# gicheonkang/gst-visdial

Hardware: AMD Instinct MI355X
Metric: dialog-rounds/sec (enc_dec_a train step) (higher is better)
Workload: dtype bf16; 1 GPU; enc_dec_a train step (fwd+loss+bwd+allreduce+AdamW, dropout on), 16 rows/GPU, seq_len 256, 37x2048 region features, answer len 25 [BASELINE configs[1] per-GPU shape]; global_batch=16, rows_per_gpu=16, seq_len=256, parallelism=dp1, hip_graph=True, optimizer_update=in the weight-gradient launch's epilogue + remainder pass, payload_written_by_wgrad_launch=False, capture_quiesce=no-process-group, full=False

## Files before the change

### gst_visdial_amd/_lib.py

```python
import ctypes as C
import os

_HERE = os.path.dirname(os.path.abspath(__file__))
LIB_PATH = os.path.join(_HERE, "lib", "libgstvd_hip.so")
ABI_VERSION = 9

F32, BF16 = 0, 1
COS_TOPK_AUTO, COS_TOPK_MANY, COS_TOPK_FEW = 0, 1, 2
EPI_BIAS, EPI_ADD, EPI_GELU, EPI_DGELU, EPI_DROPOUT = 1, 2, 4, 8, 16
EPI_COLSUM, EPI_COLSUM_ACC = 32, 64
EPI_ADAMW = 128
LN_RESID, LN_EMBED, LN_IMAGE = 0, 1, 2
RANK_MAX_OPTIONS = 128
(RANK_N_SPARSE, RANK_N_GT_SKIPPED, RANK_N_NDCG, RANK_N_NDCG_EMPTY, RANK_N_REL_SKIPPED, RANK_N_CALLS, RANK_NDCG_SUM) = range(7)
RANK_HIST = 8
RANK_ACC_SLOTS = RANK_HIST + RANK_MAX_OPTIONS + 1

_vp, _i64, _i32, _f32, _u32 = C.c_void_p, C.c_int64, C.c_int32, C.c_float, C.c_uint32


class GemmDesc(C.Structure):
    _fields_ = [("A", _vp), ("B", _vp), ("C", _vp), ("bias", _vp), ("addend", _vp), ("aux", _vp),
                ("M", _i64), ("N", _i64), ("K", _i64),
                ("lda", _i64), ("ldb", _i64), ("ldc", _i64), ("ldadd", _i64), ("ldaux", _i64),
# ... 150 lines not shown
    "gstvd_gemm_ln_bwd": (_i32, [C.POINTER(GemmDesc), C.POINTER(LnBwdDesc), _vp]),
    "gstvd_gemm_ln_rows_per_block": (_i64, []),
    "gstvd_colsum_partials": (_i32, [_vp, _i64, _i64, _i64, _vp, _vp, _vp, _i32, _vp]),
    "gstvd_colsum_batched": (_i32, [_vp, _i64, _i64, _vp]),
    "gstvd_colsum_slabs_batched": (_i32, [_vp, _i64, _i64, _i32, _vp]),
    "gstvd_colsum_slabs": (_i32, [_vp, _i64, _i64, _i64, _i32, _vp, _i64, _vp]),
    "gstvd_colsum": (_i32, [_vp, _i64, _i64, _i64, _i32, _vp, _vp, _i64, _i32, _vp]),
    "gstvd_locgrad": (_i32, [_vp, _i64, _vp, _i64, _i64, _i32, _vp, _i32, _vp]),
    "gstvd_attn_fwd": (_i32, [C.POINTER(AttnDesc), _vp]),
    "gstvd_attn_bwd": (_i32, [C.POINTER(AttnDesc), _vp]),
    "gstvd_attn_group_bwd": (_i32, [C.POINTER(AttnDesc), _vp]),
    "gstvd_ln_kernel_name": (_i32, [_vp, _i32, C.c_char_p, _i32]),
    "gstvd_attn_kernel_name": (_i32, [C.POINTER(AttnDesc), _i32, C.c_char_p, _i32]),
    "gstvd_attn_probs": (_i32, [C.POINTER(AttnDesc), _vp, _i32, _vp]),
    "gstvd_ce_fwd": (_i32, [_vp, _i64, _vp, _i64, _i64, _i64, _i32, _vp, _vp, _vp, _vp]),
    "gstvd_ce_bwd": (_i32, [_vp, _i64, _vp, _vp, _vp, _vp, _i32, _i64, _i64, _i64, _i32, _vp, _i64, _vp]),
    "gstvd_ce_bwd_rows": (_i32, [_vp, _i64, _vp, _vp, _vp, _i64, _i64, _i64, _i32, _vp, _i64, _vp]),
    "gstvd_fgsm_step": (_i32, [_vp, _vp, _f32, _vp, _i64, _vp]),
    "gstvd_answer_scores": (_i32, [_vp, _i64, _vp, _vp, _i64, _i64, _i32, _vp, _vp]),
    "gstvd_rank_loss": (_i32, [_vp, _i64, _vp, _vp, _vp, _i64, _i64, _i64, _f32, _i32, _vp, _vp, _vp, _vp, _vp, _vp]),
    "gstvd_sample_topk": (_i32, [C.POINTER(SampleDesc), _vp]),
    "gstvd_sample_topk_scored": (_i32, [C.POINTER(SampleDesc), _vp, _i64, _vp]),
    "gstvd_vl_split": (_i32, [_vp, _i64, _i64, _i64, _i64, _i32, _vp, _vp, _f32, _u32, _u32, _vp, _vp]),
    "gstvd_cast": (_i32, [_vp, _i32, _vp, _i32, _i64, _vp]),
    "gstvd_cast_ranges": (_i32, [_vp, _vp, _vp, _vp, _i64, _i64, _vp]),
    "gstvd_scale": (_i32, [_vp, _vp, _i64, _vp]),
    "gstvd_rng_advance": (_i32, [_vp, _vp]),
    "gstvd_dropout_mask": (_i32, [_vp, _i64, _f32, _u32, _vp, _vp]),
    "gstvd_adamw": (_i32, [_vp, _vp, _vp, _vp, _vp, _i64, _vp, _vp, _i64, _f32, _f32, _f32, _vp, _f32, _i64, _vp]),
    "gstvd_adamw_bf16grad": (_i32, [_vp, _vp, _i64, _vp, _vp, _vp, _i64, _vp, _vp, _i64, _f32, _f32, _f32, _vp, _f32, _i64, _vp]),
# ... 73 lines not shown
```

### gst_visdial_amd/csrc/layernorm.hip

```cpp
#include <stdio.h>

#include "common.h"

struct LnP {
  gstvd_ln_t f;
  const void* dy; int64_t lddy; void* dres; int64_t lddres; void* dx; int64_t lddx; float* partial;
  float *dword, *dpos, *dtt, *dtt_ext;
};

static inline int ln_bwd_rw(int64_t M) { return M <= 8192 ? 1 : 2; }
static inline int ln_bwd_nw(int64_t M, int mode, int64_t H) { return (M >= 2048 && mode != GSTVD_LN_EMBED && H <= 768) ? 16 : 4; }

template <typename T, int MODE>
DEVFN f32x4 ln_prologue(const gstvd_ln_t& f, int64_t row, int c, const DropKey& dpre,
                        int64_t id, int64_t tpos, int64_t seg, const float* locrow) {
  f32x4 h;
  if (MODE == GSTVD_LN_RESID) {
    h = ld4((const T*)f.x + row * f.ldx + c);
    h *= drop_factor4(dpre, (uint64_t)(row * f.H + c));
    if (f.res) h += ld4((const T*)f.res + row * f.ldres + c);
  } else if (MODE == GSTVD_LN_EMBED) {
    h = *(const f32x4*)(f.word + id * f.H + c) + *(const f32x4*)(f.pos + tpos * f.H + c);
    const float* trow = (seg < f.type_vocab) ? f.tt + seg * f.H : f.tt_ext + (seg - f.type_vocab) * f.H;
    h += *(const f32x4*)(trow + c);
// ... 521 lines not shown
  if (dtype == GSTVD_BF16) hipLaunchKernelGGL(colsum_slab_kernel<bf16>, grid, dim3(256), 0, s, (const bf16*)x, ldx, M, N, scratch);
  else if (dtype == GSTVD_F32) hipLaunchKernelGGL(colsum_slab_kernel<float>, grid, dim3(256), 0, s, (const float*)x, ldx, M, N, scratch);
  else return GSTVD_E_DTYPE;
  GSTVD_LAUNCH_CHECK();
  hipLaunchKernelGGL(colsum_final_kernel, dim3((unsigned)((N + 63) / 64)), dim3(256), 0, s, scratch, nslab, N, out, accumulate);
  GSTVD_LAUNCH_CHECK();
  return 0;
}

extern "C" int gstvd_locgrad(const void* dh, int64_t lddh, const float* loc, int64_t M, int64_t H, int32_t dtype,
                             float* dw_loc, int32_t accumulate, gstvd_stream_t stream) {
  if (!dh || !loc || !dw_loc) return GSTVD_E_NULL;
  if (M <= 0 || H <= 0) return GSTVD_E_SHAPE;
  hipStream_t s = (hipStream_t)stream;
  if (!accumulate) {
    hipError_t e = hipMemsetAsync(dw_loc, 0, (size_t)H * 5 * sizeof(float), s);
    if (e != hipSuccess) return (int)e;
  }
  dim3 grid((unsigned)((H + 255) / 256), 16);
  if (dtype == GSTVD_BF16) hipLaunchKernelGGL(locgrad_kernel<bf16>, grid, dim3(256), 0, s, (const bf16*)dh, lddh, loc, M, H, dw_loc);
  else if (dtype == GSTVD_F32) hipLaunchKernelGGL(locgrad_kernel<float>, grid, dim3(256), 0, s, (const float*)dh, lddh, loc, M, H, dw_loc);
  else return GSTVD_E_DTYPE;
  GSTVD_LAUNCH_CHECK();
  return 0;
}
```

### gst_visdial_amd/csrc/loss.hip

```cpp
#include "loss_reduce.h"
#include "ce_row.h"
#include <math.h>

template <typename T>
__global__ __launch_bounds__(256) void ce_fwd_kernel(const T* logits, int64_t ldl, const int64_t* labels, int64_t V,
                                                     int64_t ignore, float* row_loss, float* lse_out) {
  __shared__ float red[4];
  const int64_t m = blockIdx.x;
  const T* x = logits + m * ldl;
  const int64_t V4 = V & ~(int64_t)3;
  float mx = -INFINITY;
  for (int64_t c = threadIdx.x * 4; c < V4; c += 1024) {
    f32x4 v = ld4(x + c);
    mx = fmaxf(fmaxf(mx, fmaxf(v[0], v[1])), fmaxf(v[2], v[3]));
  }
  for (int64_t c = V4 + threadIdx.x; c < V; c += 256) mx = fmaxf(mx, to_f(x[c]));
  mx = block_reduce(mx, red, true);
  float s = 0.f;
  for (int64_t c = threadIdx.x * 4; c < V4; c += 1024) {
    f32x4 v = ld4(x + c);
    s += __expf(v[0] - mx) + __expf(v[1] - mx) + __expf(v[2] - mx) + __expf(v[3] - mx);
  }
  for (int64_t c = V4 + threadIdx.x; c < V; c += 256) s += __expf(to_f(x[c]) - mx);
  s = block_reduce(s, red, false);
  if (threadIdx.x == 0) {
    const float lse = mx + logf(s);
    lse_out[m] = lse;
    const int64_t lab = labels[m];
    row_loss[m] = (lab == ignore || lab < 0 || lab >= V) ? 0.f : lse - to_f(x[lab]);
  }
}

template <typename T>
__global__ __launch_bounds__(256) void ce_bwd_kernel(const T* logits, int64_t ldl, const int64_t* labels, const float* lse,
                                                     const float* stats, const float* gscale, int mean, int64_t V,
                                                     int64_t ignore, T* dl, int64_t ldd) {
  const int64_t m = blockIdx.x;
  const int64_t lab = labels[m];
  const bool keep = !(lab == ignore || lab < 0 || lab >= V);
  float gs = gscale ? gscale[0] : 1.f;
  if (mean) gs /= stats[1];
  ce_bwd_row(logits + m * ldl, dl + m * ldd, lab, keep, lse[m], gs, V, ldd);
}

template <typename T>
// ... 189 lines not shown
  GSTVD_FOR_DTYPE(dtype, E, hipLaunchKernelGGL(vl_split_kernel<E>, grid, dim3(256), 0, s, (const E*)d_enc, B, R, T, H, (E*)d_v, (E*)d_t, p, site_v, site_t, rng));
  GSTVD_LAUNCH_CHECK();
  return 0;
}

extern "C" int gstvd_abi_version(void) { return 9; }
extern "C" const char* gstvd_build_arch(void) { return "gfx950"; }

extern "C" int gstvd_ce_fwd(const void* logits, int64_t ldl, const int64_t* labels, int64_t M, int64_t V, int64_t ignore_index,
                            int32_t dtype, float* row_loss, float* lse, float* stats, gstvd_stream_t stream) {
  if (!logits || !labels || !row_loss || !lse || !stats) return GSTVD_E_NULL;
  if (M <= 0 || V <= 0 || (ldl % 4) || ldl < V) return GSTVD_E_SHAPE;
  if (dtype != GSTVD_BF16 && dtype != GSTVD_F32) return GSTVD_E_DTYPE;
  if (ce_misaligned(logits, dtype)) return GSTVD_E_ALIGN;
  hipStream_t s = (hipStream_t)stream;
  GSTVD_FOR_DTYPE(dtype, T, hipLaunchKernelGGL(ce_fwd_kernel<T>, dim3((unsigned)M), dim3(256), 0, s, (const T*)logits, ldl, labels, V, ignore_index, row_loss, lse));
  GSTVD_LAUNCH_CHECK();
  hipLaunchKernelGGL(row_loss_reduce_kernel, dim3(1), dim3(256), 0, s, (const float*)row_loss, labels, ignore_index, 0, M, stats);
  GSTVD_LAUNCH_CHECK();
  return 0;
}

extern "C" int gstvd_ce_bwd(const void* logits, int64_t ldl, const int64_t* labels, const float* lse, const float* stats,
                            const float* gscale, int32_t mean, int64_t M, int64_t V, int64_t ignore_index, int32_t dtype,
                            void* dlogits, int64_t ldd, gstvd_stream_t stream) {
  if (!logits || !labels || !lse || !stats || !dlogits) return GSTVD_E_NULL;
  if (M <= 0 || V <= 0 || (ldl % 4) || (ldd % 4) || ldl < V || ldd < V) return GSTVD_E_SHAPE;
  if (dtype != GSTVD_BF16 && dtype != GSTVD_F32) return GSTVD_E_DTYPE;
  if (ce_misaligned(logits, dtype) || ce_misaligned(dlogits, dtype)) return GSTVD_E_ALIGN;
  hipStream_t s = (hipStream_t)stream;
  GSTVD_FOR_DTYPE(dtype, T, hipLaunchKernelGGL(ce_bwd_kernel<T>, dim3((unsigned)M), dim3(256), 0, s, (const T*)logits, ldl, labels, lse, stats, gscale, mean, V, ignore_index, (T*)dlogits, ldd));
  GSTVD_LAUNCH_CHECK();
  return 0;
// ... 131 lines not shown
```

### gst_visdial_amd/csrc/loss_reduce.h

```cpp
#pragma once
#include "common.h"

static __global__ __launch_bounds__(256) void row_loss_reduce_kernel(const float* row_loss, const int64_t* labels, int64_t value, int eq,
                                                                     int64_t M, float* stats) {
  __shared__ float red[4];
  float s = 0.f, n = 0.f;
  for (int64_t i = threadIdx.x; i < M; i += blockDim.x) {
    s += row_loss[i];
    n += (!labels || (labels[i] == value) == (eq != 0)) ? 1.f : 0.f;
  }
  s = block_reduce(s, red, false);
  n = block_reduce(n, red, false);
  if (threadIdx.x == 0) { stats[0] = s; stats[1] = n; stats[2] = s / n; }
}
```

### gst_visdial_amd/engine.py

```python
import contextlib
import os
import weakref

import torch

from . import attn_maps, ops
from .config import encoder_schedule
from .engine_decode import DecodeMixin
from .engine_disc import DiscMixin, _DiscFn
from .engine_rank import RankMixin, _RankFn
from .storage import Act, Arena, FlatParams
from ._lib import GstvdError, EPI_GELU, EPI_DGELU, LN_RESID, LN_EMBED, LN_IMAGE


EARLY_WGRAD = 1

_DEVICE_STREAMS = {}


def device_streams(device):
    key = torch.device(device).index
    if key is None:
        key = torch.cuda.current_device()
    if key not in _DEVICE_STREAMS:
# ... 14 lines not shown
        self.enc_cfg, self.dec_cfg = enc_cfg, dec_cfg
        prec = params.get("amd_precision", "bf16")
        if prec not in ("bf16", "fp32"):
            raise GstvdError("params['amd_precision'] must be 'bf16' or 'fp32'")
        self.precision = prec
        self.adt = torch.bfloat16 if prec == "bf16" else torch.float32
        self.flat = None
        self.arena = None
        self.rng = None
        self._decode_sessions = {}
        self._last_decode = None
        self._early, self._early_fused = False, ()
        self.anchor = None
        self._emb_span_ok = {}
        self._first_idx, self._seeds = {}, None
        self.pipe = None
        self.tape, self.rec = [], False
        self.accumulate, self.written = False, set()
        self._maps = None
        self._inputs_only, self._io = False, False
        self.stats = {}
        self._validate = True
        self.use_streams = bool(params.get("amd_streams", True))
        self.fuse_ln = (prec == "bf16" and bool(params.get("amd_fuse_ln", True)) and os.environ.get("GSTVD_FUSE_LN", "1") != "0")
        self.tag = "t"

    @property
    def model(self):
        m = self._model_ref()
        if m is None:
# ... 36 lines not shown
                "inputs on %s but the model's parameters are on %s: gst_visdial_amd runs one process per GPU.  "
                "nn.DataParallel(model, [0]) is fine; for N GPUs launch N ranks (torchrun --nproc-per-node N) and attach "
                "pipeline.BackwardPipeline for the gradient all-reduce (INTEGRATION.md, 'Multi-GPU')" % (device, self.flat.device))
        if not self.flat.is_materialized():
            self.flat.materialize(device)
            self._bind_views()
            self._decode_sessions.clear()
        if self.arena is None or self.arena.device != device:
            self._decode_sessions.clear()
            self.arena = Arena(device)
            seed = int(self.model.params.get("amd_seed", 0))
            import torch.distributed as dist
            if dist.is_available() and dist.is_initialized() and self.model.params.get("amd_seed_per_rank", True):
                seed = ops.rank_seed(seed, dist.get_rank())
            self.rng = ops.Rng(device, seed=seed)
            self.anchor = torch.zeros(1, device=device, requires_grad=True)
            self.side, self.aux = device_streams(device)
            self.aux_busy = False
            self.colsums = ops.ColsumBatch(device)
            self.wgrads = ops.GemmGroup(device, a_km=True, b_km=True)
        self.flat.refresh_shadow()

    def _bind_views(self):
        f = self.flat
        wbuf = f.S if self.precision == "bf16" else f.P
        self.W, self.Pv, self.Gv = {}, {}, {}
        for name in f.slots:
            self.Pv[name] = f.view(f.P, name)
            if f.G is not None:
                self.Gv[name] = f.view(f.G, name)
# ... 291 lines not shown
                fresh.append(n)
            elif self.wgrads.pending_into(gv):
                self.wgrads.flush()
            tabs.append(gv)
        if len(fresh) == 4:
            lo = self.flat.slots[prefix + ".word"][0]
            hi = self.flat.slots[prefix + ".tte"][0] + tabs[3].numel()
            ok = self._emb_span_ok.get((prefix, lo, hi))
            if ok is None:
                mine = set(prefix + n for n in (".word", ".pos", ".tt", ".tte"))
                own = set(self.flat.slots[n][0] for n in mine)
                ok = hi >= lo and all(not (lo <= off < hi) or off in own for name, (off, _) in self.flat.slots.items() if name not in mine)
                self._emb_span_ok[(prefix, lo, hi)] = ok
            if not ok:
                raise GstvdError("internal: embedding tables are not contiguous in the flat buffer")
            self.flat.G[lo:hi].zero_()
        else:
            for n, gv in zip((".word", ".pos", ".tt", ".tte"), tabs):
                if n in fresh:
                    gv.zero_()
        nblk = ops.ln_bwd_blocks(M)
        partial = self.arena.alloc(nblk * 4 * H, torch.float32)
        ops.ln_bwd(kw, y.g, partial, dword=tabs[0], dpos=tabs[1], dtt=tabs[2], dtt_ext=tabs[3])
        gw, aw = self.grad_slot(prefix + ".ln.w")
        gb, ab = self.grad_slot(prefix + ".ln.b")
        tt = tabs[2]
        self.colsums.add(partial, (gw, gb, tt[0]), nblk, 4 * H, H, 3, (aw, ab, True))
        if tt.shape[0] > 1:
            self.colsums.add(partial[3 * H:], (tt[1], None, None), nblk, 4 * H, H, 1, (True, False, False))

    def img_embed(self, x, loc, cfg):
        M, H = x.M, cfg.v_hidden_size
        y = self.act(M, H)
        kw = dict(mode=LN_IMAGE, dtype=ops.dt(x.t), M=M, H=H, gamma=self.Pv["vemb.ln.w"], beta=self.Pv["vemb.ln.b"],
                  mean=self.vec(M), rstd=self.vec(M), eps=1e-12, x=x.t, y=y.t, loc=loc, w_loc=self.Pv["vemb.loc.w"],
# ... 211 lines not shown
            raise GstvdError("sequence length %d exceeds max_position_embeddings" % T)
        if segs is None:
            segs = torch.zeros_like(ids)
        if self._validate:
            if int(segs.max()) >= c.type_vocab_size + 10 or int(segs.min()) < 0:
                raise GstvdError("segment id out of range")
            if int(ids.max()) >= c.vocab_size or int(ids.min()) < 0 or int(dec_ids.max()) >= c.vocab_size or int(dec_ids.min()) < 0:
                raise GstvdError("token id out of range")
            self._validate = bool(self.model.params.get("amd_validate_inputs", False))
        I = dict(B=Bn, T=T, R=R, U=dec_ids.shape[1])
        I["ids"], I["segs"] = ids.contiguous().view(-1), segs.contiguous().view(-1)
        tm = att_mask if att_mask is not None else torch.ones(Bn, T, device=dev)
        vm = img_mask if img_mask is not None else torch.ones(Bn, R, device=dev)
        I["tmask"], I["vmask"] = tm.float().contiguous(), vm.float().contiguous()
        em = self.arena.alloc(Bn * (R + T), torch.float32, (Bn, R + T))
        em[:, :R].copy_(I["vmask"])
        em[:, R:].copy_(I["tmask"])
        I["emask"] = em
        I["dmask"] = dec_mask.float().contiguous() if dec_mask is not None else None
        I["dec_ids"] = dec_ids.contiguous().view(-1)
        f2 = feats.reshape(Bn * R, feats.shape[-1])
        if self.adt == torch.float32:
            I["feats"] = f2.float().contiguous()
        else:
            fb = self.buf(Bn * R, f2.shape[1])
            ops.cast(f2.float().contiguous(), fb)
            I["feats"] = fb
        I["loc"] = loc.reshape(Bn * R, 5).float().contiguous()
        I["feats_grad"] = bool(feats.requires_grad and torch.is_grad_enabled())
        return I

    def _refuse_maps(self, what):
        if self._maps is not None:
            raise GstvdError("%s under an attention-map request: %s" % (what, attn_maps.ALLOWED))

    def _begin(self, device, record, inference=False, maps_ok=False):
        if self._maps is not None:
            if not maps_ok:
                self._refuse_maps("this engine call")
            if self.model.training or "train" in str(self.model.params.get("mode", "")):
                self._refuse_maps("a module in training state or a 'train' mode")
            if record:
                self._refuse_maps("a forward that records its backward (wrap the call in torch.no_grad())")
            if torch.cuda.is_current_stream_capturing():
                self._refuse_maps("a stream capture (the forward of a request is issued eagerly)")
        self.prepare(device)
        self._last_decode = None
        self.arena.reset()
        self.tape, self.rec, self.tag = [], record, "t"
        self.main = torch.cuda.current_stream()
        self._site, self.site_log = 0, {}
        training = bool(self.model.training)
        self.train = training and not inference
        if training:
            self.rng.advance()

    def _shift_labels(self, dec_ids):
        dc = self.dec_cfg
        labels = dec_ids.new_zeros(dec_ids.shape)
        labels[:, :-1] = dec_ids[:, 1:].clone()
        dec_ids.masked_fill_(dec_ids == dc.eos_token_id, dc.pad_token_id)
        return labels

    def _ce(self, logits, labels, rows, U, mean=True):
        dc = self.dec_cfg
        Md, V = rows * U, dc.vocab_size
        lab = labels.contiguous().view(-1)
        row_loss, lse, stats = self.vec(Md), self.vec(Md), self.vec(4)
        ops.ce_fwd(logits.t, lab, Md, V, row_loss, lse, stats, ignore_index=dc.pad_token_id)
        ce = dict(lab=lab, row_loss=row_loss, lse=lse, stats=stats, Md=Md, V=V, pad=dc.pad_token_id)
        return (stats[2] if mean else row_loss), logits.t.view(rows, U, self.flat.Vp)[:, :, :V], ce

    def _soft_labels(self, soft, dec_ids, loss_reduction):
        if soft is None or (soft[0] is None and soft[1] is None):
            return None
        sid, slp, alpha, temperature = soft
        if sid is None or slp is None:
            raise GstvdError("dec_soft_ids and dec_soft_logp go together: both or neither")
        alpha, temperature = float(alpha), float(temperature)
        if not 0.0 <= alpha <= 1.0:
            raise GstvdError("distill_alpha = %r outside [0, 1]" % alpha)
        if not (temperature > 0.0 and temperature != float("inf")):
            raise GstvdError("distill_temperature = %r must be positive and finite" % temperature)
        Bn, U = dec_ids.shape
# ... 10 lines not shown
                    logp=slp.to(device=dev, dtype=torch.float32).contiguous().view(-1, K), alpha=alpha, temperature=temperature)

    def _distill(self, logits, ce, soft):
        Md = ce["Md"]
        row_l, row_kd, lse_tau, stats = self.vec(Md), self.vec(Md), self.vec(Md), self.vec(4)
        ops.distill_fwd(logits.t, ce["lab"], soft["ids"], soft["logp"], Md, ce["V"], soft["alpha"], soft["temperature"], ce["row_loss"],
                        row_l, row_kd, lse_tau, stats, ignore_index=ce["pad"])
        ce.update(soft=soft, lse_tau=lse_tau, row_kd=row_kd, ce_stats=ce["stats"], stats=stats, row_loss=row_l, ce_row_loss=ce["row_loss"])
        return stats[2]

    def step(self, feats, loc, img_mask, ids, segs, att_mask, dec_ids, dec_mask, labels, loss_reduction=True, soft=None, soft_top_k=None):
        record = torch.is_grad_enabled()
        soft = self._soft_labels(soft, dec_ids, loss_reduction)
        if soft_top_k is not None and (record or soft is not None or self.model.training):
            raise GstvdError("soft_top_k is the teacher's side: eval(), torch.no_grad() and no soft labels of its own")
        self._begin(ids.device, record, maps_ok=True)
        if labels is None:
            labels = self._shift_labels(dec_ids)
        I = self._inputs(feats, loc, img_mask, ids, segs, att_mask, dec_ids, dec_mask)
        if self._inputs_only and not (record and I["feats_grad"]):
            raise GstvdError("inputs_only(): the call needs enabled gradients and enc_image_features that require grad -- "
                             "d loss / d enc_image_features is all such a backward returns")
        xt, xv = self.encoder(I)
        enc = self.fusion(xt, xv, I)
        y, logits = self.decoder(enc, I)
        loss_raw, lv, ce = self._ce(logits, labels, I["B"], I["U"], loss_reduction)
        if soft_top_k is not None:
            return loss_raw.clone(), lv.to(torch.float32, copy=True), self._topk_soft(logits, ce, I["B"], I["U"], soft_top_k)
        if soft is not None:
            loss_raw = self._distill(logits, ce, soft)
        st = dict(ce, I=I, logits=logits, mean=bool(loss_reduction), tape=self.tape, inputs_only=self._inputs_only)
        self.last = dict(enc_t=xt, enc_v=xv, enc=enc, dec_hidden=y, logits=logits, lse=ce["lse"], row_loss=ce["row_loss"])
        if record:
            loss = _StepFn.apply(self.anchor, feats if I["feats_grad"] else None, self, st, loss_raw)
            return loss, lv
        return loss_raw.clone(), lv.to(torch.float32, copy=True)

    @contextlib.contextmanager
    def inputs_only(self):
        prev, self._inputs_only = self._inputs_only, True
        try:
            yield self
        finally:
            self._inputs_only = prev

    def backward(self, st, gloss):
# ... 104 lines not shown
        _, logits = self.decoder(enc, I, self._cross_kv(enc), kv_group=group)
        U = I["U"]
        tgt = dec_ids.new_zeros(dec_ids.shape)
        tgt[:, :-1] = dec_ids[:, 1:]
        ce = self._ce(logits, tgt, rows, U)[2]
        scores = torch.empty(rows, dtype=torch.float32, device=ids.device)
        ops.answer_scores(logits.t, ce["lse"], dec_ids.contiguous(), rows, U, scores)
        return scores


class _StepFn(torch.autograd.Function):

    @staticmethod
    def forward(ctx, anchor, feats, engine, st, loss_raw):
        engine._fn_enter(ctx, feats, st)
        return loss_raw.clone()

    @staticmethod
    def backward(ctx, gloss):
        return None, ctx.engine._fn_feats_grad(ctx, ctx.engine.backward(ctx.st, gloss)), None, None, None


def _owner_engine(module, kind):
    eng = getattr(module, "_standalone_engine", None)
    if eng is None:
        raise GstvdError("%s.forward outside an EncoderDecoderModel is not supported by the MI355X engine; "
                         "call EncoderDecoderModel(...) (the reference scripts only ever do that)" % kind)
    return eng


def standalone_encoder_forward(module, input_ids, image_feat, image_loc, token_type_ids, attention_mask, image_attention_mask):
# ... 56 lines not shown
```

### gst_visdial_amd/ops.py

```python
import ctypes as C

import torch

from . import _lib as L
from ._lib import F32, BF16, EPI_BIAS, EPI_ADD, EPI_GELU, EPI_DGELU, EPI_DROPOUT, LN_RESID, LN_EMBED, LN_IMAGE

_DT = {torch.float32: F32, torch.bfloat16: BF16}


def dt(t):
    return _DT[t.dtype]


def _p(t):
    if t is None:
        return None
    if not t.is_cuda:
        raise L.GstvdError("gst_visdial_amd ops need GPU tensors (got %s); there is no CPU path" % t.device)
    return t.data_ptr()


_RAW_STREAM = getattr(torch._C, "_cuda_getCurrentRawStream", None)
_DEV_INDEX = None

# ... 150 lines not shown


def splitk_plan(dtype_in, M, N, K, batch, a_km, b_km):
    if not SPLITK or dtype_in != BF16 or batch != 1 or (a_km and not b_km):
        return 1
    if M <= 16 and not a_km and not b_km:
        return 1
    if M >= 256 and N >= 128 and ((M + 127) // 128) * ((N + 127) // 128) >= 96:
        return 1
    tiles = ((M + 63) // 64) * ((N + 63) // 64)
    nkt = (K + 63) // 64
    s = min(256 // max(tiles, 1), nkt // 10, 8)
    return s if s >= 2 else 1


def _splitk_scratch(device):
    key = (device.index, torch.cuda.current_stream().cuda_stream)
    ws = _SPLITK_WS.get(key)
    if ws is None:
        ws = torch.zeros(4096 + 256 * 64 * 64 * 4, dtype=torch.uint8, device=device)
        _SPLITK_WS[key] = ws
    return ws


GROUP_ORDER = 3
N_XCD = 8
XCD_CUS = 32
GROUP_ORDER_MIN_TILES = 4 * N_XCD * 32


def xcd_block_map(shapes, tile, fused_epilogue, mode=1, unit_tiles=40):
    T = tile
    if mode not in (1, 3):
        raise ValueError("xcd_block_map: mode 1 (queues of whole units) or 3 (rounds with short-K fillers)")
    rounds = mode == 3
# ... 468 lines not shown
    a.lddk = dK.stride(-2) if lddk is None else lddk
    a.lddv = dV.stride(-2) if lddv is None else lddv
    e0 = _prof_begin()
    L.check("gstvd_attn_group_bwd", lib.gstvd_attn_group_bwd(C.byref(a), _stream()))
    _prof_end(e0, "attn_group_bwd_d%d" % a.d, 14.0 * a.B * a.nh * a.Lq * a.Lk * a.d, 0.0, (a.B, a.nh, a.Lq, a.Lk, a.kv_group))


def ce_fwd(logits, labels, M, V, row_loss, lse, stats, ignore_index=0):
    lib = L.load()
    e0 = _prof_begin()
    L.check("gstvd_ce_fwd", lib.gstvd_ce_fwd(_p(logits), logits.stride(-2), _p(labels), M, V, ignore_index, dt(logits),
                                             _p(row_loss), _p(lse), _p(stats), _stream()))
    _prof_end(e0, "ce_fwd", 0.0, float(M) * V * logits.element_size(), (M, V))


def ce_bwd(logits, labels, lse, stats, gscale, mean, M, V, dlogits, ignore_index=0):
    lib = L.load()
    e0 = _prof_begin()
    L.check("gstvd_ce_bwd", lib.gstvd_ce_bwd(_p(logits), logits.stride(-2), _p(labels), _p(lse), _p(stats), _p(gscale),
                                             int(mean), M, V, ignore_index, dt(logits), _p(dlogits), dlogits.stride(-2),
                                             _stream()))
    _prof_end(e0, "ce_bwd", 0.0, float(M) * V * (logits.element_size() + dlogits.element_size()), (M, V))


def ce_bwd_rows(logits, labels, lse, g, M, V, dlogits, ignore_index=0):
    lib = L.load()
    if g.dtype != torch.float32 or not g.is_contiguous() or g.numel() != M:
        raise L.GstvdError("ce_bwd_rows: g must be a contiguous fp32 tensor of %d elements" % M)
    if dlogits.dtype != logits.dtype:
        raise L.GstvdError("ce_bwd_rows: logits and dlogits must share one dtype")
# ... 967 lines not shown
```

### gst_visdial_amd/optim.py

```python
import torch

from . import ops

NO_DECAY = ("bias", "LayerNorm.bias", "LayerNorm.weight")


def warmup_linear_nonzero(step, warmup_steps, t_total, base_lr, min_lr=1e-5):
    if step < warmup_steps:
        f = float(step) / float(max(1, warmup_steps))
    else:
        f = max(0, float(t_total - step) / float(max(1.0, t_total - warmup_steps)))
    return base_lr * f if base_lr * f > min_lr else min_lr


def reference_param_index(model):
    dec_mod = model.decoder.decoder
    if dec_mod.bert.embeddings is not model.encoder.bert_pretrained.bert.embeddings:
        raise NotImplementedError("reference optimizer state is defined for the train_gen.py set-up: share the embeddings "
                                  "first (decoder.decoder.bert.embeddings = encoder.bert_pretrained.bert.embeddings)")
    out = [("encoder." + k, p) for k, p in model.encoder.named_parameters()]
    lm_w = dec_mod.lm_head.decoder.weight
    for k, p in model.decoder.named_parameters():
        if p is lm_w:
            continue
# ... 143 lines not shown
        key = (lr_t, lr_i)
        if key == self._last_lr_key:
            return
        for i, (lr, wd, live) in enumerate(self.base):
            cur = 0.0 if not live else (lr_t if lr == self.lr else lr_i)
            self.hp_host[2 * i] = cur
            self.hp_host[2 * i + 1] = wd
        self.hp.copy_(self.hp_host, non_blocking=True)
        self._last_lr_key = key

    def begin_step(self):
        if not self._ensure_built():
            raise RuntimeError("FusedAdamW before the first forward")
        self._upload_hp()
        self.opt_step += 1
        self.step_dev.add_(1.0)

    def apply_range(self, lo, hi, grad_bf16=None, fused=(), grad_origin=None):
        flat = self.engine.flat
        if fused:
            if grad_bf16 is not None:
                raise ValueError("a fused weight-gradient update and a compressed gradient slice exclude each other")
            blocks, skip = self._remainder(lo, hi, fused)
            if blocks.numel():
                ops.adamw_blocks(flat.P, flat.G, self.m, self.v, flat.S, self.seg_end, self.hp, self.step_dev, blocks, skip,
                                 self.betas[0], self.betas[1], self.eps, self.grad_scale, begin=lo, end=hi)
        elif grad_bf16 is not None:
            ops.adamw(flat.P, grad_bf16, self.m, self.v, flat.S, self.seg_end, self.hp, self.step_dev, self.betas[0],
                      self.betas[1], self.eps, self.grad_scale, begin=lo, end=hi, grad_origin=lo if grad_origin is None else grad_origin)
        else:
            ops.adamw(flat.P, flat.G, self.m, self.v, flat.S, self.seg_end, self.hp, self.step_dev, self.betas[0],
# ... 141 lines not shown
```

### include/gstvd_hip.h

```cpp
#ifndef GSTVD_HIP_H
#define GSTVD_HIP_H

#include <stdint.h>

#ifdef __cplusplus
extern "C" {
#endif

typedef void* gstvd_stream_t;

enum { GSTVD_F32 = 0, GSTVD_BF16 = 1 };
enum {
  GSTVD_E_DTYPE = -1, GSTVD_E_SHAPE = -2, GSTVD_E_ALIGN = -3, GSTVD_E_NULL = -4, GSTVD_E_UNSUPPORTED = -5
};

int gstvd_abi_version(void);
const char* gstvd_build_arch(void);

enum { GSTVD_EPI_BIAS = 1, GSTVD_EPI_ADD = 2, GSTVD_EPI_GELU = 4, GSTVD_EPI_DGELU = 8, GSTVD_EPI_DROPOUT = 16,
       GSTVD_EPI_COLSUM = 32, GSTVD_EPI_COLSUM_ACC = 64,
       GSTVD_EPI_ADAMW = 128 };

typedef struct {
  const void* A; const void* B; void* C;
// ... 84 lines not shown
  void *dQ, *dK, *dV; int64_t lddq, lddk, lddv;
  float* delta;
  int32_t kv_group;
  int32_t q_bstride, kv_bstride;
  uint64_t* drop_bits;
} gstvd_attn_t;
int gstvd_attn_fwd(const gstvd_attn_t* a, gstvd_stream_t s);
int gstvd_attn_bwd(const gstvd_attn_t* a, gstvd_stream_t s);
int gstvd_attn_kernel_name(const gstvd_attn_t* a, int32_t bwd, char* buf, int32_t buf_len);
int gstvd_attn_group_bwd(const gstvd_attn_t* a, gstvd_stream_t s);
int gstvd_attn_probs(const gstvd_attn_t* a, float* P, int32_t head_mean, gstvd_stream_t s);

int gstvd_ce_fwd(const void* logits, int64_t ldl, const int64_t* labels, int64_t M, int64_t V,
                 int64_t ignore_index, int32_t dtype, float* row_loss, float* lse, float* stats,
                 gstvd_stream_t s);
int gstvd_ce_bwd(const void* logits, int64_t ldl, const int64_t* labels, const float* lse,
                 const float* stats, const float* gscale, int32_t mean, int64_t M, int64_t V,
                 int64_t ignore_index, int32_t dtype, void* dlogits, int64_t ldd, gstvd_stream_t s);
int gstvd_ce_bwd_rows(const void* logits, int64_t ldl, const int64_t* labels, const float* lse, const float* g, int64_t M,
                      int64_t V, int64_t ignore_index, int32_t dtype, void* dlogits, int64_t ldd, gstvd_stream_t s);
int gstvd_fgsm_step(const float* x, const float* g, float eps, float* out, int64_t n, gstvd_stream_t s);
int gstvd_answer_scores(const void* logits, int64_t ldl, const float* lse, const int64_t* dec_ids,
                        int64_t rows, int64_t U, int32_t dtype, float* scores, gstvd_stream_t s);
int gstvd_rank_loss(const void* logits, int64_t ldl, const float* lse, const int64_t* dec_ids, const float* relevance,
                    int64_t E, int64_t G, int64_t U, float inv_temperature, int32_t dtype, float* scores, float* p,
                    float* round_loss, float* g_tok, float* stats, gstvd_stream_t s);

typedef struct {
  const void* logits; int64_t ld; int32_t dtype; int32_t B; int32_t V; int32_t top_k; float temperature;
  const float* u; int64_t* out; int64_t out_stride; const uint8_t* banned; int64_t banned_ld;
  const int64_t* hist; int64_t hist_ld; int32_t hist_T; int32_t ngram;
  const int64_t* ids_tm; int64_t ids_stride; int32_t cur_len; int32_t n_special; int32_t special[8];
  float top_p; int32_t reserved_;
} gstvd_sample_t;
int gstvd_sample_topk(const gstvd_sample_t* a, gstvd_stream_t s);
int gstvd_sample_topk_scored(const gstvd_sample_t* a, float* logp, int64_t logp_stride, gstvd_stream_t s);

int gstvd_vl_split(const void* d_enc, int64_t B, int64_t R, int64_t T, int64_t H, int32_t dtype, void* d_v, void* d_t,
                   float p, uint32_t site_v, uint32_t site_t, const uint64_t* rng, gstvd_stream_t s);

int gstvd_cast(const void* src, int32_t src_dtype, void* dst, int32_t dst_dtype, int64_t n, gstvd_stream_t s);
int gstvd_cast_ranges(const float* src, void* dst_bf16, const int64_t* ranges_dev, const int32_t* blk0_dev, int64_t nranges,
                      int64_t total_blocks, gstvd_stream_t s);
int gstvd_scale(float* x, const float* factor, int64_t n, gstvd_stream_t s);
int gstvd_rng_advance(uint64_t* rng, gstvd_stream_t s);
int gstvd_dropout_mask(float* out, int64_t n, float p, uint32_t site, const uint64_t* rng, gstvd_stream_t s);

int gstvd_adamw(float* param, const float* grad, float* m, float* v, void* shadow_bf16, int64_t n,
                const int64_t* seg_end, const float* hp, int64_t nseg, float beta1, float beta2, float eps,
                const float* step , float grad_scale, int64_t begin, gstvd_stream_t s);
int gstvd_adamw_bf16grad(float* param, const void* grad_bf16, int64_t grad_origin, float* m, float* v, void* shadow_bf16,
                         int64_t n, const int64_t* seg_end, const float* hp, int64_t nseg, float beta1, float beta2, float eps,
                         const float* step, float grad_scale, int64_t begin, gstvd_stream_t s);

int gstvd_adamw_blocks(float* param, const float* grad, float* m, float* v, void* shadow_bf16, int64_t n,
                       const int64_t* seg_end, const float* hp, int64_t nseg, float beta1, float beta2, float eps,
                       const float* step, float grad_scale, int64_t begin, const int32_t* block_list_dev, int64_t nblocks,
                       const uint8_t* seg_skip_dev, gstvd_stream_t s);

typedef struct {
// ... 174 lines not shown
```

Before: 1340 dialog-rounds/sec.

## Cut small launches: fuse step-begin ops, last-block CE loss reduce, kernel zeroing

Measured after the change: 1335 dialog-rounds/sec. About the same (-0.3%).

```diff
diff --git a/gst_visdial_amd/_lib.py b/gst_visdial_amd/_lib.py
--- a/gst_visdial_amd/_lib.py
+++ b/gst_visdial_amd/_lib.py
@@ -188,6 +188,10 @@
     "gstvd_attn_kernel_name": (_i32, [C.POINTER(AttnDesc), _i32, C.c_char_p, _i32]),
     "gstvd_attn_probs": (_i32, [C.POINTER(AttnDesc), _vp, _i32, _vp]),
     "gstvd_ce_fwd": (_i32, [_vp, _i64, _vp, _i64, _i64, _i64, _i32, _vp, _vp, _vp, _vp]),
+    "gstvd_ce_fwd_reduce": (_i32, [_vp, _i64, _vp, _i64, _i64, _i64, _i32, _vp, _vp, _vp, _vp, _vp, _vp]),
+    "gstvd_step_begin": (_i32, [_vp, _vp, _vp, _vp, _i64, _i64, _i64, _vp, _vp, _i64, _vp]),
+    "gstvd_zero_span": (_i32, [_vp, _i64, _vp]),
+    "gstvd_counter_add": (_i32, [_vp, _f32, _vp]),
     "gstvd_ce_bwd": (_i32, [_vp, _i64, _vp, _vp, _vp, _vp, _i32, _i64, _i64, _i64, _i32, _vp, _i64, _vp]),
     "gstvd_ce_bwd_rows": (_i32, [_vp, _i64, _vp, _vp, _vp, _i64, _i64, _i64, _i32, _vp, _i64, _vp]),
     "gstvd_fgsm_step": (_i32, [_vp, _vp, _f32, _vp, _i64, _vp]),
diff --git a/gst_visdial_amd/csrc/layernorm.hip b/gst_visdial_amd/csrc/layernorm.hip
--- a/gst_visdial_amd/csrc/layernorm.hip
+++ b/gst_visdial_amd/csrc/layernorm.hip
@@ -559,8 +559,13 @@
   if (M <= 0 || H <= 0) return GSTVD_E_SHAPE;
   hipStream_t s = (hipStream_t)stream;
   if (!accumulate) {
-    hipError_t e = hipMemsetAsync(dw_loc, 0, (size_t)H * 5 * sizeof(float), s);
-    if (e != hipSuccess) return (int)e;
+    if (((uintptr_t)dw_loc & 15) == 0) {
+      const int rc = gstvd_zero_span(dw_loc, H * 5, stream);
+      if (rc) return rc;
+    } else {
+      hipError_t e = hipMemsetAsync(dw_loc, 0, (size_t)H * 5 * sizeof(float), s);
+      if (e != hipSuccess) return (int)e;
+    }
   }
   dim3 grid((unsigned)((H + 255) / 256), 16);
   if (dtype == GSTVD_BF16) hipLaunchKernelGGL(locgrad_kernel<bf16>, grid, dim3(256), 0, s, (const bf16*)dh, lddh, loc, M, H, dw_loc);
diff --git a/gst_visdial_amd/csrc/loss.hip b/gst_visdial_amd/csrc/loss.hip
--- a/gst_visdial_amd/csrc/loss.hip
+++ b/gst_visdial_amd/csrc/loss.hip
@@ -4,8 +4,10 @@
 
 template <typename T>
 __global__ __launch_bounds__(256) void ce_fwd_kernel(const T* logits, int64_t ldl, const int64_t* labels, int64_t V,
-                                                     int64_t ignore, float* row_loss, float* lse_out) {
+                                                     int64_t ignore, float* row_loss, float* lse_out, int64_t M, float* stats,
+                                                     float* loss_out, int* counter) {
   __shared__ float red[4];
+  __shared__ int arrived;
   const int64_t m = blockIdx.x;
   const T* x = logits + m * ldl;
   const int64_t V4 = V & ~(int64_t)3;
@@ -27,8 +29,17 @@
     const float lse = mx + logf(s);
     lse_out[m] = lse;
     const int64_t lab = labels[m];
-    row_loss[m] = (lab == ignore || lab < 0 || lab >= V) ? 0.f : lse - to_f(x[lab]);
-  }
+    const float rl = (lab == ignore || lab < 0 || lab >= V) ? 0.f : lse - to_f(x[lab]);
+    if (!counter) { row_loss[m] = rl; return; }
+    __hip_atomic_store(row_loss + m, rl, __ATOMIC_RELAXED, __HIP_MEMORY_SCOPE_AGENT);
+    asm volatile("s_waitcnt vmcnt(0)" ::: "memory");
+    arrived = __hip_atomic_fetch_add(counter, 1, __ATOMIC_RELAXED, __HIP_MEMORY_SCOPE_AGENT);
+  }
+  if (!counter) return;
+  __syncthreads();
+  if (arrived != (int)gridDim.x - 1) return;
+  if (threadIdx.x == 0) __hip_atomic_store(counter, 0, __ATOMIC_RELAXED, __HIP_MEMORY_SCOPE_AGENT);
+  row_loss_reduce_rows<true>(row_loss, labels, ignore, 0, M, stats, loss_out, red);
 }
 
 template <typename T>
@@ -248,9 +259,24 @@
   if (dtype != GSTVD_BF16 && dtype != GSTVD_F32) return GSTVD_E_DTYPE;
   if (ce_misaligned(logits, dtype)) return GSTVD_E_ALIGN;
   hipStream_t s = (hipStream_t)stream;
-  GSTVD_FOR_DTYPE(dtype, T, hipLaunchKernelGGL(ce_fwd_kernel<T>, dim3((unsigned)M), dim3(256), 0, s, (const T*)logits, ldl, labels, V, ignore_index, row_loss, lse));
+  GSTVD_FOR_DTYPE(dtype, T, hipLaunchKernelGGL(ce_fwd_kernel<T>, dim3((unsigned)M), dim3(256), 0, s, (const T*)logits, ldl, labels, V, ignore_index, row_loss, lse,
+                                               M, (float*)nullptr, (float*)nullptr, (int*)nullptr));
   GSTVD_LAUNCH_CHECK();
   hipLaunchKernelGGL(row_loss_reduce_kernel, dim3(1), dim3(256), 0, s, (const float*)row_loss, labels, ignore_index, 0, M, stats);
+  GSTVD_LAUNCH_CHECK();
+  return 0;
+}
+
+extern "C" int gstvd_ce_fwd_reduce(const void* logits, int64_t ldl, const int64_t* labels, int64_t M, int64_t V, int64_t ignore_index,
+                                   int32_t dtype, float* row_loss, float* lse, float* stats, float* loss_out, int32_t* counter,
+                                   gstvd_stream_t stream) {
+  if (!logits || !labels || !row_loss || !lse || !stats || !counter) return GSTVD_E_NULL;
+  if (M <= 0 || M > 0x7fffffff || V <= 0 || (ldl % 4) || ldl < V) return GSTVD_E_SHAPE;
+  if (dtype != GSTVD_BF16 && dtype != GSTVD_F32) return GSTVD_E_DTYPE;
+  if (ce_misaligned(logits, dtype) || ((uintptr_t)counter & 3)) return GSTVD_E_ALIGN;
+  hipStream_t s = (hipStream_t)stream;
+  GSTVD_FOR_DTYPE(dtype, T, hipLaunchKernelGGL(ce_fwd_kernel<T>, dim3((unsigned)M), dim3(256), 0, s, (const T*)logits, ldl, labels, V, ignore_index, row_loss, lse,
+                                               M, stats, loss_out, (int*)counter));
   GSTVD_LAUNCH_CHECK();
   return 0;
 }
diff --git a/gst_visdial_amd/csrc/loss_reduce.h b/gst_visdial_amd/csrc/loss_reduce.h
--- a/gst_visdial_amd/csrc/loss_reduce.h
+++ b/gst_visdial_amd/csrc/loss_reduce.h
@@ -1,15 +1,25 @@
 #pragma once
 #include "common.h"
+
+template <bool AGENT>
+DEVFN void row_loss_reduce_rows(const float* row_loss, const int64_t* labels, int64_t value, int eq, int64_t M, float* stats,
+                                float* loss_out, float* red) {
+  float s = 0.f, n = 0.f;
+  for (int64_t i = threadIdx.x; i < M; i += blockDim.x) {
+    if constexpr (AGENT) s += __hip_atomic_load(row_loss + i, __ATOMIC_RELAXED, __HIP_MEMORY_SCOPE_AGENT);
+    else s += row_loss[i];
+    n += (!labels || (labels[i] == value) == (eq != 0)) ? 1.f : 0.f;
+  }
+  s = block_reduce(s, red, false);
+  n = block_reduce(n, red, false);
+  if (threadIdx.x == 0) {
+    stats[0] = s; stats[1] = n; stats[2] = s / n;
+    if (loss_out) loss_out[0] = s / n;
+  }
+}
 
 static __global__ __launch_bounds__(256) void row_loss_reduce_kernel(const float* row_loss, const int64_t* labels, int64_t value, int eq,
                                                                      int64_t M, float* stats) {
   __shared__ float red[4];
-  float s = 0.f, n = 0.f;
-  for (int64_t i = threadIdx.x; i < M; i += blockDim.x) {
-    s += row_loss[i];
-    n += (!labels || (labels[i] == value) == (eq != 0)) ? 1.f : 0.f;
-  }
-  s = block_reduce(s, red, false);
-  n = block_reduce(n, red, false);
-  if (threadIdx.x == 0) { stats[0] = s; stats[1] = n; stats[2] = s / n; }
+  row_loss_reduce_rows<false>(row_loss, labels, value, eq, M, stats, nullptr, red);
 }
diff --git a/gst_visdial_amd/csrc/step_edge.hip b/gst_visdial_amd/csrc/step_edge.hip
--- /dev/null
+++ b/gst_visdial_amd/csrc/step_edge.hip
@@ -0,0 +1,69 @@
+#include "common.h"
+#include "../../include/gstvd_hip.h"
+
+__global__ __launch_bounds__(256) void step_begin_kernel(uint64_t* rng, const float* vmask, const float* tmask, float* emask, int64_t B,
+                                                         int64_t R, int64_t T, const float* feats, bf16* feats_out, int64_t n,
+                                                         int64_t cast_blocks) {
+  const int64_t blk = blockIdx.x;
+  if (rng && blk == 0 && threadIdx.x == 0) rng[1] += 1;
+  if (blk < cast_blocks) {
+    const int64_t i = (blk * 256 + threadIdx.x) * 4;
+    if (i + 3 < n) st4(feats_out + i, ld4(feats + i));
+    else for (int64_t j = i; j < n; ++j) feats_out[j] = from_f<bf16>(to_f(feats[j]));
+    return;
+  }
+  if (!emask) return;
+  const int64_t S = R + T, e = (blk - cast_blocks) * 256 + threadIdx.x;
+  if (e >= B * S) return;
+  const int64_t b = e / S, c = e - b * S;
+  emask[e] = c < R ? vmask[b * R + c] : tmask[b * T + (c - R)];
+}
+
+__global__ __launch_bounds__(256) void zero_span_kernel(float* p, int64_t n4, int64_t n) {
+  const f32x4 z = {0.f, 0.f, 0.f, 0.f};
+  const int64_t v0 = (int64_t)blockIdx.x * 1024 + threadIdx.x;
+#pragma unroll
+  for (int v = 0; v < 4; ++v) {
+    const int64_t k = v0 + v * 256;
+    if (k < n4) st4(p + k * 4, z);
+  }
+  if (blockIdx.x == 0 && threadIdx.x < (n & 3)) p[n4 * 4 + threadIdx.x] = 0.f;
+}
+
+extern "C" int gstvd_step_begin(uint64_t* rng, const float* vmask, const float* tmask, float* emask, int64_t B, int64_t R, int64_t T,
+                                const float* feats, void* feats_bf16, int64_t n_feats, gstvd_stream_t stream) {
+  const bool masks = emask != nullptr && B > 0 && R + T > 0, cast = feats_bf16 != nullptr && n_feats > 0;
+  if (emask && (B < 0 || R < 0 || T < 0)) return GSTVD_E_SHAPE;
+  if (masks && ((R > 0 && !vmask) || (T > 0 && !tmask))) return GSTVD_E_NULL;
+  if (feats_bf16 && n_feats < 0) return GSTVD_E_SHAPE;
+  if (cast && !feats) return GSTVD_E_NULL;
+  if (cast && (((uintptr_t)feats | (uintptr_t)feats_bf16) & 15)) return GSTVD_E_ALIGN;
+  if (!rng && !masks && !cast) return 0;
+  const int64_t cast_blocks = cast ? (n_feats + 1023) / 1024 : 0, mask_blocks = masks ? (B * (R + T) + 255) / 256 : 0;
+  const int64_t blocks = cast_blocks + mask_blocks > 0 ? cast_blocks + mask_blocks : 1;
+  if (blocks > 0x7fffffff) return GSTVD_E_SHAPE;
+  hipLaunchKernelGGL(step_begin_kernel, dim3((unsigned)blocks), dim3(256), 0, (hipStream_t)stream, rng, vmask, tmask, masks ? emask : nullptr,
+                     B, R, T, feats, (bf16*)feats_bf16, cast ? n_feats : 0, cast_blocks);
+  GSTVD_LAUNCH_CHECK();
+  return 0;
+}
+
+__global__ void counter_add_kernel(float* x, float v) { x[0] += v; }
+
+extern "C" int gstvd_counter_add(float* x, float v, gstvd_stream_t stream) {
+  if (!x) return GSTVD_E_NULL;
+  hipLaunchKernelGGL(counter_add_kernel, dim3(1), dim3(1), 0, (hipStream_t)stream, x, v);
+  GSTVD_LAUNCH_CHECK();
+  return 0;
+}
+
+extern "C" int gstvd_zero_span(float* p, int64_t n, gstvd_stream_t stream) {
+  if (!p) return GSTVD_E_NULL;
+  if (n <= 0) return GSTVD_E_SHAPE;
+  if ((uintptr_t)p & 15) return GSTVD_E_ALIGN;
+  const int64_t n4 = n / 4, blocks = (n4 + 1023) / 1024 > 0 ? (n4 + 1023) / 1024 : 1;
+  if (blocks > 0x7fffffff) return GSTVD_E_SHAPE;
+  hipLaunchKernelGGL(zero_span_kernel, dim3((unsigned)blocks), dim3(256), 0, (hipStream_t)stream, p, n4, n);
+  GSTVD_LAUNCH_CHECK();
+  return 0;
+}
diff --git a/gst_visdial_amd/engine.py b/gst_visdial_amd/engine.py
--- a/gst_visdial_amd/engine.py
+++ b/gst_visdial_amd/engine.py
@@ -52,6 +52,7 @@
         self.anchor = None
         self._emb_span_ok = {}
         self._first_idx, self._seeds = {}, None
+        self._rng_due = False
         self.pipe = None
         self.tape, self.rec = [], False
         self.accumulate, self.written = False, set()
@@ -118,6 +119,7 @@
             if dist.is_available() and dist.is_initialized() and self.model.params.get("amd_seed_per_rank", True):
                 seed = ops.rank_seed(seed, dist.get_rank())
             self.rng = ops.Rng(device, seed=seed)
+            self.ce_counter = torch.zeros(1, dtype=torch.int32, device=device)
             self.anchor = torch.zeros(1, device=device, requires_grad=True)
             self.side, self.aux = device_streams(device)
             self.aux_busy = False
@@ -439,11 +441,11 @@
                 self._emb_span_ok[(prefix, lo, hi)] = ok
             if not ok:
                 raise GstvdError("internal: embedding tables are not contiguous in the flat buffer")
-            self.flat.G[lo:hi].zero_()
+            ops.zero_span(self.flat.G[lo:hi])
         else:
             for n, gv in zip((".word", ".pos", ".tt", ".tte"), tabs):
                 if n in fresh:
-                    gv.zero_()
+                    ops.zero_span(gv)
         nblk = ops.ln_bwd_blocks(M)
         partial = self.arena.alloc(nblk * 4 * H, torch.float32)
         ops.ln_bwd(kw, y.g, partial, dword=tabs[0], dpos=tabs[1], dtt=tabs[2], dtt_ext=tabs[3])
@@ -685,17 +687,17 @@
         vm = img_mask if img_mask is not None else torch.ones(Bn, R, device=dev)
         I["tmask"], I["vmask"] = tm.float().contiguous(), vm.float().contiguous()
         em = self.arena.alloc(Bn * (R + T), torch.float32, (Bn, R + T))
-        em[:, :R].copy_(I["vmask"])
-        em[:, R:].copy_(I["tmask"])
         I["emask"] = em
         I["dmask"] = dec_mask.float().contiguous() if dec_mask is not None else None
         I["dec_ids"] = dec_ids.contiguous().view(-1)
-        f2 = feats.reshape(Bn * R, feats.shape[-1])
+        f2 = feats.reshape(Bn * R, feats.shape[-1]).float().contiguous()
+        rng, self._rng_due = (self.rng if self._rng_due else None), False
         if self.adt == torch.float32:
-            I["feats"] = f2.float().contiguous()
+            I["feats"] = f2
+            ops.step_begin(rng, I["vmask"], I["tmask"], em)
         else:
             fb = self.buf(Bn * R, f2.shape[1])
-            ops.cast(f2.float().contiguous(), fb)
+            ops.step_begin(rng, I["vmask"], I["tmask"], em, f2, fb)
             I["feats"] = fb
         I["loc"] = loc.reshape(Bn * R, 5).float().contiguous()
         I["feats_grad"] = bool(feats.requires_grad and torch.is_grad_enabled())
@@ -705,7 +707,7 @@
         if self._maps is not None:
             raise GstvdError("%s under an attention-map request: %s" % (what, attn_maps.ALLOWED))
 
-    def _begin(self, device, record, inference=False, maps_ok=False):
+    def _begin(self, device, record, inference=False, maps_ok=False, defer_rng=False):
         if self._maps is not None:
             if not maps_ok:
                 self._refuse_maps("this engine call")
@@ -723,7 +725,8 @@
         self._site, self.site_log = 0, {}
         training = bool(self.model.training)
         self.train = training and not inference
-        if training:
+        self._rng_due = training and defer_rng
+        if training and not defer_rng:
             self.rng.advance()
 
     def _shift_labels(self, dec_ids):
@@ -733,12 +736,15 @@
         dec_ids.masked_fill_(dec_ids == dc.eos_token_id, dc.pad_token_id)
         return labels
 
-    def _ce(self, logits, labels, rows, U, mean=True):
+    def _ce(self, logits, labels, rows, U, mean=True, loss_out=None):
         dc = self.dec_cfg
         Md, V = rows * U, dc.vocab_size
         lab = labels.contiguous().view(-1)
         row_loss, lse, stats = self.vec(Md), self.vec(Md), self.vec(4)
-        ops.ce_fwd(logits.t, lab, Md, V, row_loss, lse, stats, ignore_index=dc.pad_token_id)
+        if loss_out is not None:
+            ops.ce_fwd_reduce(logits.t, lab, Md, V, row_loss, lse, stats, self.ce_counter, loss_out, ignore_index=dc.pad_token_id)
+        else:
+            ops.ce_fwd(logits.t, lab, Md, V, row_loss, lse, stats, ignore_index=dc.pad_token_id)
         ce = dict(lab=lab, row_loss=row_loss, lse=lse, stats=stats, Md=Md, V=V, pad=dc.pad_token_id)
         return (stats[2] if mean else row_loss), logits.t.view(rows, U, self.flat.Vp)[:, :, :V], ce
 
@@ -779,7 +785,7 @@
         soft = self._soft_labels(soft, dec_ids, loss_reduction)
         if soft_top_k is not None and (record or soft is not None or self.model.training):
             raise GstvdError("soft_top_k is the teacher's side: eval(), torch.no_grad() and no soft labels of its own")
-        self._begin(ids.device, record, maps_ok=True)
+        self._begin(ids.device, record, maps_ok=True, defer_rng=True)
         if labels is None:
             labels = self._shift_labels(dec_ids)
         I = self._inputs(feats, loc, img_mask, ids, segs, att_mask, dec_ids, dec_mask)
@@ -789,12 +795,14 @@
         xt, xv = self.encoder(I)
         enc = self.fusion(xt, xv, I)
         y, logits = self.decoder(enc, I)
-        loss_raw, lv, ce = self._ce(logits, labels, I["B"], I["U"], loss_reduction)
+        own = bool(record and loss_reduction and soft is None and soft_top_k is None)
+        loss_own = torch.empty((), dtype=torch.float32, device=ids.device) if own else None
+        loss_raw, lv, ce = self._ce(logits, labels, I["B"], I["U"], loss_reduction, loss_out=loss_own)
         if soft_top_k is not None:
             return loss_raw.clone(), lv.to(torch.float32, copy=True), self._topk_soft(logits, ce, I["B"], I["U"], soft_top_k)
         if soft is not None:
             loss_raw = self._distill(logits, ce, soft)
-        st = dict(ce, I=I, logits=logits, mean=bool(loss_reduction), tape=self.tape, inputs_only=self._inputs_only)
+        st = dict(ce, I=I, logits=logits, mean=bool(loss_reduction), tape=self.tape, inputs_only=self._inputs_only, loss_own=loss_own)
         self.last = dict(enc_t=xt, enc_v=xv, enc=enc, dec_hidden=y, logits=logits, lse=ce["lse"], row_loss=ce["row_loss"])
         if record:
             loss = _StepFn.apply(self.anchor, feats if I["feats_grad"] else None, self, st, loss_raw)
@@ -929,7 +937,8 @@
     @staticmethod
     def forward(ctx, anchor, feats, engine, st, loss_raw):
         engine._fn_enter(ctx, feats, st)
-        return loss_raw.clone()
+        own = st.get("loss_own")
+        return own.detach() if own is not None else loss_raw.clone()
 
     @staticmethod
     def backward(ctx, gloss):
diff --git a/gst_visdial_amd/ops.py b/gst_visdial_amd/ops.py
--- a/gst_visdial_amd/ops.py
+++ b/gst_visdial_amd/ops.py
@@ -188,11 +188,23 @@
     return s if s >= 2 else 1
 
 
+_SPLITK_WS_BYTES = 4096 + 256 * 64 * 64 * 4
+_SPLITK_POOL = {}
+_SPLITK_POOL_SLOTS = 8
+
+
 def _splitk_scratch(device):
     key = (device.index, torch.cuda.current_stream().cuda_stream)
     ws = _SPLITK_WS.get(key)
     if ws is None:
-        ws = torch.zeros(4096 + 256 * 64 * 64 * 4, dtype=torch.uint8, device=device)
+        pool = _SPLITK_POOL.get(device.index)
+        if (pool is None or pool[1] == _SPLITK_POOL_SLOTS) and not torch.cuda.is_current_stream_capturing():
+            pool = _SPLITK_POOL[device.index] = [torch.zeros(_SPLITK_POOL_SLOTS * _SPLITK_WS_BYTES, dtype=torch.uint8, device=device), 0]
+        if pool is None or pool[1] == _SPLITK_POOL_SLOTS:
+            ws = torch.zeros(_SPLITK_WS_BYTES, dtype=torch.uint8, device=device)
+        else:
+            ws = pool[0][pool[1] * _SPLITK_WS_BYTES:(pool[1] + 1) * _SPLITK_WS_BYTES]
+            pool[1] += 1
         _SPLITK_WS[key] = ws
     return ws
 
@@ -691,6 +703,52 @@
     _prof_end(e0, "ce_fwd", 0.0, float(M) * V * logits.element_size(), (M, V))
 
 
+def ce_fwd_reduce(logits, labels, M, V, row_loss, lse, stats, counter, loss_out=None, ignore_index=0):
+    if counter.dtype != torch.int32 or counter.numel() < 1:
+        raise L.GstvdError("ce_fwd_reduce: counter must be an int32 tensor")
+    if loss_out is not None and (loss_out.dtype != torch.float32 or loss_out.numel() < 1):
+        raise L.GstvdError("ce_fwd_reduce: loss_out must be an fp32 tensor")
+    lib = L.load()
+    e0 = _prof_begin()
+    L.check("gstvd_ce_fwd_reduce", lib.gstvd_ce_fwd_reduce(_p(logits), logits.stride(-2), _p(labels), M, V, ignore_index, dt(logits),
+                                                           _p(row_loss), _p(lse), _p(stats), _p(loss_out), _p(counter), _stream()))
+    _prof_end(e0, "ce_fwd", 0.0, float(M) * V * logits.element_size(), (M, V))
+
+
+def step_begin(rng=None, vmask=None, tmask=None, emask=None, feats=None, feats_out=None):
+    B = R = T = n = 0
+    if emask is not None:
+        B, S = emask.shape
+        R = vmask.shape[1] if vmask is not None else 0
+        T = tmask.shape[1] if tmask is not None else 0
+        for m, w in ((vmask, R), (tmask, T), (emask, R + T)):
+            if m is not None and (m.dtype != torch.float32 or not m.is_contiguous() or tuple(m.shape) != (B, w)):
+                raise L.GstvdError("step_begin: masks must be contiguous fp32 [B, R], [B, T] and [B, R + T]")
+        if S != R + T:
+            raise L.GstvdError("step_begin: emask has %d columns for R + T = %d" % (S, R + T))
+    if feats_out is not None:
+        n = feats.numel()
+        if (feats.dtype != torch.float32 or feats_out.dtype != torch.bfloat16 or feats_out.numel() != n
+                or not feats.is_contiguous() or not feats_out.is_contiguous()):
+            raise L.GstvdError("step_begin: feats must be contiguous fp32 and feats_out contiguous bf16 of the same size")
+    lib = L.load()
+    L.check("gstvd_step_begin", lib.gstvd_step_begin(rng.ptr() if rng is not None else None, _p(vmask), _p(tmask), _p(emask), B, R, T,
+                                                     _p(feats), _p(feats_out), n, _stream()))
+
+
+def counter_add(x, v):
+    if x.dtype != torch.float32 or x.numel() < 1:
+        raise L.GstvdError("counter_add: an fp32 tensor")
+    L.check("gstvd_counter_add", L.load().gstvd_counter_add(_p(x), float(v), _stream()))
+
+
+def zero_span(t):
+    if t.dtype != torch.float32 or not t.is_contiguous():
+        raise L.GstvdError("zero_span: a contiguous fp32 tensor")
+    if t.numel():
+        L.check("gstvd_zero_span", L.load().gstvd_zero_span(_p(t), t.numel(), _stream()))
+
+
 def ce_bwd(logits, labels, lse, stats, gscale, mean, M, V, dlogits, ignore_index=0):
     lib = L.load()
     e0 = _prof_begin()
diff --git a/gst_visdial_amd/optim.py b/gst_visdial_amd/optim.py
--- a/gst_visdial_amd/optim.py
+++ b/gst_visdial_amd/optim.py
@@ -181,7 +181,7 @@
             raise RuntimeError("FusedAdamW before the first forward")
         self._upload_hp()
         self.opt_step += 1
-        self.step_dev.add_(1.0)
+        ops.counter_add(self.step_dev, 1.0)
 
     def apply_range(self, lo, hi, grad_bf16=None, fused=(), grad_origin=None):
         flat = self.engine.flat
diff --git a/include/gstvd_hip.h b/include/gstvd_hip.h
--- a/include/gstvd_hip.h
+++ b/include/gstvd_hip.h
@@ -122,6 +122,9 @@
 int gstvd_ce_fwd(const void* logits, int64_t ldl, const int64_t* labels, int64_t M, int64_t V,
                  int64_t ignore_index, int32_t dtype, float* row_loss, float* lse, float* stats,
                  gstvd_stream_t s);
+int gstvd_ce_fwd_reduce(const void* logits, int64_t ldl, const int64_t* labels, int64_t M, int64_t V,
+                        int64_t ignore_index, int32_t dtype, float* row_loss, float* lse, float* stats, float* loss_out,
+                        int32_t* counter, gstvd_stream_t s);
 int gstvd_ce_bwd(const void* logits, int64_t ldl, const int64_t* labels, const float* lse,
                  const float* stats, const float* gscale, int32_t mean, int64_t M, int64_t V,
                  int64_t ignore_index, int32_t dtype, void* dlogits, int64_t ldd, gstvd_stream_t s);
@@ -152,6 +155,10 @@
                       int64_t total_blocks, gstvd_stream_t s);
 int gstvd_scale(float* x, const float* factor, int64_t n, gstvd_stream_t s);
 int gstvd_rng_advance(uint64_t* rng, gstvd_stream_t s);
+int gstvd_step_begin(uint64_t* rng, const float* vmask, const float* tmask, float* emask, int64_t B, int64_t R, int64_t T,
+                     const float* feats, void* feats_bf16, int64_t n_feats, gstvd_stream_t s);
+int gstvd_counter_add(float* x, float v, gstvd_stream_t s);
+int gstvd_zero_span(float* p, int64_t n, gstvd_stream_t s);
 int gstvd_dropout_mask(float* out, int64_t n, float p, uint32_t site, const uint64_t* rng, gstvd_stream_t s);
 
 int gstvd_adamw(float* param, const float* grad, float* m, float* v, void* shadow_bf16, int64_t n,
```
